# littlemesie/recommend-tf2.0

Measured on NVIDIA B200. Metric: DLRM train samples/sec, higher is better.
Workload: dtype f32

## Files before the change

recommend-tf2.0_b200/csrc/embed_bwd.cu:

```cuda
#include <cstdlib>

#include "rtf_common.cuh"

namespace rtf {

struct BwdParams {
  float* w[RTF_MAX_FIELDS];
  float* s1[RTF_MAX_FIELDS];
  float* s2[RTF_MAX_FIELDS];
  long long rows[RTF_MAX_FIELDS];
  int dim[RTF_MAX_FIELDS];
  int field_table[RTF_MAX_FIELDS];
  int field_off[RTF_MAX_FIELDS];
  int n_tables, n_fields, sumD, row_bits, L, pool;
  long long grad_sb;
  rtf_opt opt;
};

template <typename IdT>
__global__ void __launch_bounds__(256)
make_keys(const __grid_constant__ BwdParams P, const IdT* __restrict__ ids, long long n,
          long long sb, long long sf, long long sl, uint32_t* __restrict__ keys) {
  const long long p = (long long)blockIdx.x * blockDim.x + threadIdx.x;
  if (p >= n) return;
  const int F = P.n_fields;
  const long long LF = (long long)P.L * F;
  const long long b = p / LF;
  const int r = (int)(p - b * LF);
  const int l = r / F;
  const int f = r - l * F;
  const int t = P.field_table[f];
  const long long id = (long long)__ldg(ids + b * sb + (long long)f * sf + (long long)l * sl);
  uint32_t key;
  if (id < 0 || id >= P.rows[t])
    key = (uint32_t)P.n_tables << P.row_bits;
  else
    key = ((uint32_t)t << P.row_bits) | (uint32_t)id;
  keys[p] = key;
}

constexpr int SCAN_THREADS = 256;
constexpr int SCAN_ITEMS = 8;
constexpr int SCAN_TILE = SCAN_THREADS * SCAN_ITEMS;

template <typename T>
__device__ __forceinline__ T block_exclusive_scan(T v, T* total) {
  __shared__ T warp_tot[SCAN_THREADS / 32];
  const int lane = threadIdx.x & 31, wid = threadIdx.x >> 5;
  T inc = v;
#pragma unroll
  for (int o = 1; o < 32; o <<= 1) {
    T y = __shfl_up_sync(0xffffffffu, inc, o);
    if (lane >= o) inc += y;
  }
  if (lane == 31) warp_tot[wid] = inc;
  __syncthreads();
  T base = 0, tot = 0;
#pragma unroll
  for (int w = 0; w < SCAN_THREADS / 32; ++w) {
    const T t = warp_tot[w];
    if (w < wid) base += t;
    tot += t;
  }
  __syncthreads();
  *total = tot;
  return base + inc - v;
}

template <typename T, typename In>
__global__ void __launch_bounds__(SCAN_THREADS)
scan_tile_reduce(In in, long long n, T* __restrict__ tile_sums) {
  const long long base = (long long)blockIdx.x * SCAN_TILE + (long long)threadIdx.x * SCAN_ITEMS;
  T s = 0;
#pragma unroll
  for (int k = 0; k < SCAN_ITEMS; ++k)
    if (base + k < n) s += in(base + k);
  T tot;
  block_exclusive_scan<T>(s, &tot);
  if (threadIdx.x == 0) tile_sums[blockIdx.x] = tot;
}

template <typename T>
__global__ void __launch_bounds__(1024) scan_tile_sums(T* __restrict__ tile_sums, int nt) {
  __shared__ T wsum[32];
  __shared__ T carry_s;
  if (threadIdx.x == 0) carry_s = 0;
  __syncthreads();
  const int lane = threadIdx.x & 31, wid = threadIdx.x >> 5;
  for (int base = 0; base < nt; base += 1024) {
    const int i = base + threadIdx.x;
    const T v = i < nt ? tile_sums[i] : 0;
    T inc = v;
#pragma unroll
    for (int o = 1; o < 32; o <<= 1) {
      T y = __shfl_up_sync(0xffffffffu, inc, o);
      if (lane >= o) inc += y;
    }
    if (lane == 31) wsum[wid] = inc;
    __syncthreads();
    if (wid == 0) {
      T w = wsum[lane], winc = w;
#pragma unroll
      for (int o = 1; o < 32; o <<= 1) {
        T y = __shfl_up_sync(0xffffffffu, winc, o);
        if (lane >= o) winc += y;
      }
      wsum[lane] = winc - w;
    }
    __syncthreads();
    const T carry = carry_s;
    const T excl = carry + wsum[wid] + inc - v;
    if (i < nt) tile_sums[i] = excl;
    __syncthreads();
    if (threadIdx.x == 1023) carry_s = excl + v;
    __syncthreads();
  }
}

template <typename T, typename In, typename Out>
__global__ void __launch_bounds__(SCAN_THREADS)
scan_tile_apply(In in, Out out, long long n, const T* __restrict__ tile_sums) {
  const long long base = (long long)blockIdx.x * SCAN_TILE + (long long)threadIdx.x * SCAN_ITEMS;
  T v[SCAN_ITEMS];
  T s = 0;
#pragma unroll
  for (int k = 0; k < SCAN_ITEMS; ++k) {
    v[k] = base + k < n ? in(base + k) : 0;
    s += v[k];
  }
  T tot;
  T ex = block_exclusive_scan<T>(s, &tot) + tile_sums[blockIdx.x];
#pragma unroll
  for (int k = 0; k < SCAN_ITEMS; ++k) {
    if (base + k < n) out(base + k, ex, v[k]);
    ex += v[k];
  }
}

struct InArray {
  const uint32_t* a;
  __device__ uint32_t operator()(long long i) const { return a[i]; }
};
struct OutArray {
  uint32_t* a;
  __device__ void operator()(long long i, uint32_t ex, uint32_t) const { a[i] = ex; }
};
struct InHeadFlag {
  const uint32_t* keys;
  __device__ uint32_t operator()(long long i) const {
    return (i == 0 || keys[i] != keys[i - 1]) ? 1u : 0u;
  }
};
struct OutSegments {
  const uint32_t* keys;
  uint32_t* seg_start;
  int32_t* counters;
  int32_t* d_num_uniq;
  long long n;
  uint32_t sentinel_table;
  int row_bits;
  __device__ void operator()(long long i, uint32_t ex, uint32_t flag) const {
    if (flag) seg_start[ex] = (uint32_t)i;
    if (i == n - 1) {
      const uint32_t nseg = ex + flag;
      seg_start[nseg] = (uint32_t)n;
      const int valid = (int)nseg - ((keys[i] >> row_bits) == sentinel_table ? 1 : 0);
      counters[0] = (int)nseg;
      counters[1] = valid;
      if (d_num_uniq) *d_num_uniq = valid;
    }
  }
};

struct InSegKinds {
  const uint32_t* seg_start;
  const int32_t* counters;
  __device__ unsigned long long operator()(long long i) const {
    if (i >= counters[1]) return 0ull;
    const uint32_t len = seg_start[i + 1] - seg_start[i];
    if (len <= RTF_SEG_CHUNK) return 1ull;
    return (unsigned long long)((len + RTF_SEG_CHUNK - 1) / RTF_SEG_CHUNK) << 32;
  }
};
struct OutItems {
  const uint32_t* keys;
  const uint32_t* vals;
  const uint32_t* seg_start;
  int32_t* counters;
  uint4* items;
  uint32_t* short_seg;
  uint2* long_seg;
  uint32_t* arrive;
  uint32_t cap_chunk;
  __device__ void operator()(long long i, unsigned long long ex, unsigned long long v) const {
    const int n_valid = counters[1];
    if (i >= n_valid) return;
    const uint32_t start = seg_start[i], len = seg_start[i + 1] - start;
    const uint32_t key = keys[start];
    if (v & 0xffffffffull) {
      const uint32_t j = (uint32_t)ex;
      items[cap_chunk + j] = make_uint4(key, start, len, vals[start]);
      short_seg[j] = (uint32_t)i;
    } else {
      const uint32_t nch = (uint32_t)(v >> 32), slot0 = (uint32_t)(ex >> 32);
      long_seg[slot0] = make_uint2((uint32_t)i, nch);
      for (uint32_t c = 0; c < nch; ++c) {
        const uint32_t s = start + c * RTF_SEG_CHUNK;
        arrive[slot0 + c] = 0u;
        items[slot0 + c] = make_uint4(key, s, min((uint32_t)RTF_SEG_CHUNK, start + len - s), slot0);
      }
    }
    if (i == n_valid - 1) {
      const unsigned long long tot = ex + v;
      counters[2] = (int)(uint32_t)tot;
      counters[3] = (int)(uint32_t)(tot >> 32);
    }
  }
};

template <typename T, typename In, typename Out>
static int exclusive_scan(In in, Out out, long long n, T* tile_sums, cudaStream_t st) {
  const long long nt = (n + SCAN_TILE - 1) / SCAN_TILE;
  scan_tile_reduce<T, In><<<(unsigned)nt, SCAN_THREADS, 0, st>>>(in, n, tile_sums);
  scan_tile_sums<T><<<1, 1024, 0, st>>>(tile_sums, (int)nt);
  scan_tile_apply<T, In, Out><<<(unsigned)nt, SCAN_THREADS, 0, st>>>(in, out, n, tile_sums);
  RTF_CHECK_LAUNCH();
  return 0;
}

constexpr int SORT_THREADS = 256;
constexpr int SORT_WARPS = SORT_THREADS / 32;
constexpr int SORT_ITEMS = 16;
constexpr int SORT_TILE = SORT_THREADS * SORT_ITEMS;
constexpr int SORT_MAX_BITS = 10;
constexpr int SORT_MAX_BINS = 1 << SORT_MAX_BITS;

__global__ void __launch_bounds__(SORT_THREADS)
sort_hist(const uint32_t* __restrict__ keys, long long n, int shift, int bits,
          uint32_t* __restrict__ hist, int nblk) {
  __shared__ uint32_t sh[SORT_MAX_BINS];
  const int bins = 1 << bits;
  const uint32_t mask = (uint32_t)bins - 1u;
  for (int i = threadIdx.x; i < bins; i += SORT_THREADS) sh[i] = 0;
  __syncthreads();
  const long long base = (long long)blockIdx.x * SORT_TILE;
#pragma unroll
  for (int r = 0; r < SORT_ITEMS; ++r) {
    const long long i = base + r * SORT_THREADS + threadIdx.x;
    if (i < n) atomicAdd(&sh[(keys[i] >> shift) & mask], 1u);
  }
  __syncthreads();
  for (int d = threadIdx.x; d < bins; d += SORT_THREADS)
    hist[(long long)d * nblk + blockIdx.x] = sh[d];
}

__global__ void __launch_bounds__(SORT_THREADS)
sort_scatter(const uint32_t* __restrict__ keys_in, const uint32_t* __restrict__ vals_in,
             uint32_t* __restrict__ keys_out, uint32_t* __restrict__ vals_out, long long n,
             int shift, int bits, const uint32_t* __restrict__ hist_scanned, int nblk,
             int iota_vals) {
  __shared__ uint32_t whist[SORT_WARPS][SORT_MAX_BINS];
  const int bins = 1 << bits;
  const uint32_t mask = (uint32_t)bins - 1u;
  for (int i = threadIdx.x; i < SORT_WARPS * SORT_MAX_BINS; i += SORT_THREADS)
    (&whist[0][0])[i] = 0;
  __syncthreads();
  const int lane = threadIdx.x & 31, wid = threadIdx.x >> 5;
  const uint32_t lt_mask = (1u << lane) - 1u;
  const long long wbase = (long long)blockIdx.x * SORT_TILE + (long long)wid * (32 * SORT_ITEMS);
  uint32_t k[SORT_ITEMS], v[SORT_ITEMS], rank[SORT_ITEMS];
#pragma unroll
  for (int r = 0; r < SORT_ITEMS; ++r) {
    const long long i = wbase + r * 32 + lane;
    const bool valid = i < n;
    k[r] = valid ? keys_in[i] : 0xffffffffu;
    v[r] = valid ? (iota_vals ? (uint32_t)i : vals_in[i]) : 0u;
    const uint32_t vmask = __ballot_sync(0xffffffffu, valid);
    rank[r] = 0;
    if (valid) {
      const uint32_t d = (k[r] >> shift) & mask;
      const uint32_t m = __match_any_sync(vmask, d);
      const uint32_t prior = whist[wid][d];
      __syncwarp(vmask);
      if ((m & lt_mask) == 0) whist[wid][d] = prior + __popc(m);
      __syncwarp(vmask);
      rank[r] = prior + __popc(m & lt_mask);
    }
  }
  __syncthreads();
  for (int d = threadIdx.x; d < bins; d += SORT_THREADS) {
    uint32_t run = hist_scanned[(long long)d * nblk + blockIdx.x];
#pragma unroll
    for (int w = 0; w < SORT_WARPS; ++w) {
      const uint32_t c = whist[w][d];
      whist[w][d] = run;
      run += c;
    }
  }
  __syncthreads();
#pragma unroll
  for (int r = 0; r < SORT_ITEMS; ++r) {
    const long long i = wbase + r * 32 + lane;
    if (i < n) {
      const uint32_t d = (k[r] >> shift) & mask;
      const uint32_t pos = whist[wid][d] + rank[r];
      keys_out[pos] = k[r];
      vals_out[pos] = v[r];
    }
  }
}

template <int VEC>
struct Vec {
  float v[VEC];
};
template <int VEC>
__device__ __forceinline__ Vec<VEC> vload(const float* p) {
  Vec<VEC> r;
  if constexpr (VEC == 4) {
    const float4 t = *reinterpret_cast<const float4*>(p);
    r.v[0] = t.x; r.v[1] = t.y; r.v[2] = t.z; r.v[3] = t.w;
  } else {
    r.v[0] = *p;
  }
  return r;
}
template <int VEC>
__device__ __forceinline__ Vec<VEC> vload_stream(const float* p) {
  Vec<VEC> r;
  if constexpr (VEC == 4) {
    const float4 t = ldg_nc_f4(p);
    r.v[0] = t.x; r.v[1] = t.y; r.v[2] = t.z; r.v[3] = t.w;
  } else {
    r.v[0] = __ldg(p);
  }
  return r;
}
template <int VEC>
__device__ __forceinline__ void vstore(float* p, const Vec<VEC>& a) {
  if constexpr (VEC == 4)
    *reinterpret_cast<float4*>(p) = make_float4(a.v[0], a.v[1], a.v[2], a.v[3]);
  else
    *p = a.v[0];
}

__device__ __forceinline__ const float* grad_row(const BwdParams& P, const float* grad,
                                                 uint32_t p) {
  const int F = P.n_fields;
  const uint32_t LF = (uint32_t)P.L * (uint32_t)F;
  const uint32_t b = p / LF;
  const uint32_t r = p - b * LF;
  const uint32_t l = r / (uint32_t)F;
  const uint32_t f = r - l * (uint32_t)F;
  const long long lo = P.pool == RTF_POOL_NONE ? (long long)l * P.sumD : 0;
  return grad + (long long)b * P.grad_sb + lo + P.field_off[f];
}

template <int VEC, int G, int VPL>
__device__ __forceinline__ void sum_rows(const BwdParams& P, const float* __restrict__ grad,
                                         const uint32_t* __restrict__ vals, uint32_t start,
                                         uint32_t end, bool have_first, uint32_t first_pos, int nv,
                                         int lg, float scale, Vec<VEC> (&acc)[VPL]) {
  constexpr int U = 4;
#pragma unroll 1
  for (uint32_t j0 = start; j0 < end; j0 += U) {
    const float* src[U];
#pragma unroll
    for (int u = 0; u < U; ++u) {
      src[u] = nullptr;
      if (j0 + u < end) {
        const uint32_t p = (have_first && j0 + u == start) ? first_pos : __ldg(vals + j0 + u);
        src[u] = grad_row(P, grad, p);
      }
    }
    Vec<VEC> x[U][VPL];
#pragma unroll
    for (int u = 0; u < U; ++u)
#pragma unroll
      for (int k = 0; k < VPL; ++k) {
        const int vi = lg + k * G;
        if (src[u] && vi < nv) x[u][k] = vload_stream<VEC>(src[u] + VEC * vi);
      }
#pragma unroll
    for (int u = 0; u < U; ++u)
      if (src[u]) {
#pragma unroll
        for (int k = 0; k < VPL; ++k) {
          const int vi = lg + k * G;
          if (vi < nv) {
#pragma unroll
// ... 197 lines not shown
  for (int k = 0; k < VPL; ++k)
#pragma unroll
    for (int e = 0; e < VEC; ++e) acc[k].v[e] = 0.f;
  if (i >= n_chunk) {
    RowState<VEC, VPL> st;
    if (len <= 2) {
      load_row_state<VEC, G, VPL>(P, key, nv, lg, st);
      const float* r0 = grad_row(P, grad, rec.w);
      const float* r1 = len == 2 ? grad_row(P, grad, __ldg(S.vals + start + 1)) : nullptr;
      Vec<VEC> x0[VPL], x1[VPL];
#pragma unroll
      for (int k = 0; k < VPL; ++k) {
        const int vi = lg + k * G;
        if (vi < nv) {
          x0[k] = vload_stream<VEC>(r0 + VEC * vi);
          if (r1) x1[k] = vload_stream<VEC>(r1 + VEC * vi);
        }
      }
#pragma unroll
      for (int k = 0; k < VPL; ++k) {
        const int vi = lg + k * G;
        if (vi < nv) {
#pragma unroll
          for (int e = 0; e < VEC; ++e) {
            float g = x0[k].v[e];
            if (P.pool == RTF_POOL_MEAN) g = __fmul_rn(g, scale);
            acc[k].v[e] = __fadd_rn(acc[k].v[e], g);
            if (r1) {
              float h = x1[k].v[e];
              if (P.pool == RTF_POOL_MEAN) h = __fmul_rn(h, scale);
              acc[k].v[e] = __fadd_rn(acc[k].v[e], h);
            }
          }
        }
      }
    } else {
      sum_rows<VEC, G, VPL>(P, grad, S.vals, start, start + len, true, rec.w, nv, lg, scale, acc);
      load_row_state<VEC, G, VPL>(P, key, nv, lg, st);
    }
    uint32_t seg = 0;
    if (S.uniq_key || S.uniq_grad) seg = __ldg(S.short_seg + (i - n_chunk));
    finish_row<VEC, G, VPL>(P, key, seg, nv, lg, acc, st, S.uniq_key, S.uniq_grad, S.dim_max);
    return;
  }
  const int g0 = (int)(threadIdx.x & 31) / G * G;
  const uint32_t gmask = G == 32 ? 0xffffffffu : (((1u << (G & 31)) - 1u) << g0);
  const uint32_t slot0 = rec.w;
  sum_rows<VEC, G, VPL>(P, grad, S.vals, start, start + len, false, 0u, nv, lg, scale, acc);
#pragma unroll
  for (int k = 0; k < VPL; ++k) {
    const int vi = lg + k * G;
    if (vi < nv) vstore<VEC>(S.partials + (long long)i * S.dim_max + VEC * vi, acc[k]);
  }
  __threadfence();
  __syncwarp(gmask);
  const uint2 ls = __ldg(S.long_seg + slot0);
  if (ls.y <= RTF_SEG_GROUP) {
    uint32_t ticket = 0;
    if (lg == 0) ticket = atomicAdd(S.arrive + slot0, 1u);
    ticket = __shfl_sync(gmask, ticket, g0);
    if (ticket != ls.y - 1) return;
  }
  combine_long<VEC, G, VPL>(P, S, key, slot0, i - slot0, ls, nv, lg, gmask, g0);
}

template <int VEC, int G, int VPL, int MINB>
static int launch_apply(const BwdParams& P, const SegWork& S, const float* grad,
                        long long max_items, cudaStream_t st) {
  const long long blocks = (max_items * G + 255) / 256;
  seg_apply<VEC, G, VPL, MINB><<<(unsigned)blocks, 256, 0, st>>>(P, S, grad);
  RTF_CHECK_LAUNCH();
  return 0;
}

template <int VEC, int G, int VPL>
static int launch_segments(const BwdParams& P, const SegWork& S, const float* grad,
                           long long max_items, cudaStream_t st) {
  return launch_apply<VEC, G, VPL, (VPL == 1 ? 8 : 4)>(P, S, grad, max_items, st);
}

static inline size_t align_up(size_t x, size_t a) { return (x + a - 1) / a * a; }

struct WsLayout {
  size_t keys0, keys1, vals0, vals1, hist, tile_sums, seg_start, counters, items, short_seg,
      long_seg, arrive, partials, total;
  size_t cap_chunk;
};
static WsLayout ws_layout(long long n, int dim_max) {
  WsLayout w;
  const size_t nn = (size_t)(n > 0 ? n : 1);
  const size_t nblk = (nn + SORT_TILE - 1) / SORT_TILE;
  size_t o = 0;
  auto take = [&](size_t bytes) { size_t r = o; o = align_up(o + bytes, 256); return r; };
  w.keys0 = take(nn * 4);
  w.keys1 = take(nn * 4);
  w.vals0 = take(nn * 4);
  w.vals1 = take(nn * 4);
  w.hist = take((size_t)SORT_MAX_BINS * nblk * 4);
  const size_t scan_n = nn > (size_t)SORT_MAX_BINS * nblk ? nn : (size_t)SORT_MAX_BINS * nblk;
  w.tile_sums = take(((scan_n + SCAN_TILE - 1) / SCAN_TILE + 1) * 8);
  w.seg_start = take((nn + 1) * 4);
  w.counters = take(16);
  w.cap_chunk = 2 * nn / RTF_SEG_CHUNK + 4;
  w.items = take((w.cap_chunk + nn) * 16);
  w.short_seg = take(nn * 4);
  w.long_seg = take(w.cap_chunk * 8);
  w.arrive = take(w.cap_chunk * 4);
  w.partials = take(w.cap_chunk * (size_t)dim_max * 4);
  w.total = o;
  return w;
}

}

extern "C" int rtf_embed_bwd_workspace(int64_t n_lookups, int dim_max, size_t* bytes) {
  if (!bytes || n_lookups < 0 || dim_max <= 0) return RTF_E_ARG;
  *bytes = rtf::ws_layout(n_lookups, dim_max).total;
  return 0;
}

static int embed_bwd_impl(int phase, float* const* weights, float* const* state1,
                          float* const* state2, const int64_t* rows, const int32_t* dims,
                          int n_tables, const int32_t* field_table, int n_fields,
                          const void* d_ids, int ids_i64, int64_t B, int L, int64_t ids_sb,
                          int64_t ids_sf, int64_t ids_sl, int pool, const float* d_grad,
                          int64_t grad_sb, const rtf_opt* opt, uint32_t* d_uniq_key,
                          float* d_uniq_grad, int32_t* d_num_uniq, int* row_bits_out,
                          void* d_workspace, size_t workspace_bytes, void* stream) {
  using namespace rtf;
  static const rtf_opt kNoOpt = {RTF_OPT_NONE, 0.f, 0.f, 0.f, 0.f, 0.f, nullptr};
  static float* const kNoPtrs[RTF_MAX_FIELDS] = {};
  if (!(phase & 2)) {
    opt = &kNoOpt;
    weights = kNoPtrs;
    state1 = state2 = nullptr;
  }
  if (!weights || !rows || !dims || !field_table || !opt) return RTF_E_ARG;
  if (n_tables <= 0 || n_fields <= 0 || B < 0 || L <= 0) return RTF_E_ARG;
  if (B > 0 && !d_workspace) return RTF_E_ARG;
  if (B > 0 && (phase & 1) && !d_ids) return RTF_E_ARG;
  if (B > 0 && (phase & 2) && !d_grad) return RTF_E_ARG;
  if (n_tables > RTF_MAX_FIELDS || n_fields > RTF_MAX_FIELDS) return RTF_E_RANGE;
  if (pool < RTF_POOL_NONE || pool > RTF_POOL_MEAN) return RTF_E_ARG;
  if (opt->kind < RTF_OPT_NONE || opt->kind > RTF_OPT_ADAM) return RTF_E_ARG;
  cudaStream_t st = (cudaStream_t)stream;

  BwdParams P;
  long long rows_max = 1;
  int dim_max = 0;
  bool vec_ok = ((uintptr_t)d_grad % 16 == 0) && (grad_sb % 4 == 0) &&
                (!d_uniq_grad || (uintptr_t)d_uniq_grad % 16 == 0);
  for (int t = 0; t < n_tables; ++t) {
    if (rows[t] <= 0 || dims[t] <= 0) return RTF_E_ARG;
    P.w[t] = weights[t];
    P.s1[t] = state1 ? state1[t] : nullptr;
    P.s2[t] = state2 ? state2[t] : nullptr;
    P.rows[t] = rows[t];
    P.dim[t] = dims[t];
    if (opt->kind != RTF_OPT_NONE && !P.w[t]) return RTF_E_ARG;
    if (opt->kind >= RTF_OPT_ADAGRAD && !P.s1[t]) return RTF_E_ARG;
    if (opt->kind == RTF_OPT_ADAM && !P.s2[t]) return RTF_E_ARG;
    if (dims[t] % 4 || (uintptr_t)P.w[t] % 16 || (uintptr_t)P.s1[t] % 16 ||
        (uintptr_t)P.s2[t] % 16)
      vec_ok = false;
    if (rows[t] > rows_max) rows_max = rows[t];
    if (dims[t] > dim_max) dim_max = dims[t];
  }
  int off = 0;
  for (int f = 0; f < n_fields; ++f) {
    const int t = field_table[f];
    if (t < 0 || t >= n_tables) return RTF_E_ARG;
    P.field_table[f] = t;
    P.field_off[f] = off;
    if (off % 4) vec_ok = false;
    off += dims[t];
  }
  P.sumD = off;
  if (off % 4) vec_ok = false;
  int row_bits = 1;
  while (((long long)1 << row_bits) < rows_max) ++row_bits;
  int table_bits = 1;
  while ((1 << table_bits) < n_tables + 1) ++table_bits;
  if (row_bits + table_bits > 32) return RTF_E_RANGE;
  if (row_bits_out) *row_bits_out = row_bits;
  P.n_tables = n_tables;
  P.n_fields = n_fields;
  P.row_bits = row_bits;
  P.L = L;
  P.pool = pool;
  P.grad_sb = grad_sb;
  P.opt = *opt;

  const long long n = B * (long long)L * n_fields;
  if (n >= 0x7fffffffLL) return RTF_E_RANGE;
  if (n == 0) {
    if (d_num_uniq) cudaMemsetAsync(d_num_uniq, 0, 4, st);
    return 0;
  }
  if (dim_max > (vec_ok ? 512 : 128)) return RTF_E_RANGE;
  const WsLayout W = ws_layout(n, dim_max);
  if (workspace_bytes < W.total) return RTF_E_WORKSPACE;
  if ((uintptr_t)d_workspace % 256) return RTF_E_ALIGN;
  char* ws = (char*)d_workspace;
  uint32_t* keys[2] = {(uint32_t*)(ws + W.keys0), (uint32_t*)(ws + W.keys1)};
  uint32_t* vals[2] = {(uint32_t*)(ws + W.vals0), (uint32_t*)(ws + W.vals1)};
  uint32_t* hist = (uint32_t*)(ws + W.hist);
  uint32_t* tile_sums = (uint32_t*)(ws + W.tile_sums);
  uint32_t* seg_start = (uint32_t*)(ws + W.seg_start);
  int32_t* counters = (int32_t*)(ws + W.counters);

  const int nblk = (int)((n + SORT_TILE - 1) / SORT_TILE);
  const int total_bits = row_bits + table_bits;
  const int npass = (total_bits + SORT_MAX_BITS - 1) / SORT_MAX_BITS;
  const int bits = (total_bits + npass - 1) / npass;
  int cur = npass & 1;
  if (phase & 1) {
  cur = 0;
  const unsigned kb = (unsigned)((n + 255) / 256);
  if (ids_i64)
    make_keys<int64_t><<<kb, 256, 0, st>>>(P, (const int64_t*)d_ids, n, ids_sb, ids_sf, ids_sl,
                                           keys[0]);
  else
    make_keys<int32_t><<<kb, 256, 0, st>>>(P, (const int32_t*)d_ids, n, ids_sb, ids_sf, ids_sl,
                                           keys[0]);
  RTF_CHECK_LAUNCH();

  for (int shift = 0, pass = 0; pass < npass; shift += bits, ++pass) {
    sort_hist<<<nblk, SORT_THREADS, 0, st>>>(keys[cur], n, shift, bits, hist, nblk);
    int rc = exclusive_scan<uint32_t>(InArray{hist}, OutArray{hist}, (long long)(1 << bits) * nblk,
                                      tile_sums, st);
    if (rc) return rc;
    sort_scatter<<<nblk, SORT_THREADS, 0, st>>>(keys[cur], vals[cur], keys[cur ^ 1],
                                                vals[cur ^ 1], n, shift, bits, hist, nblk,
                                                pass == 0);
    RTF_CHECK_LAUNCH();
    cur ^= 1;
  }

  cudaError_t ce = cudaMemsetAsync(counters, 0, 16, st);
  if (ce != cudaSuccess) return (int)ce;
  {
    OutSegments outseg{keys[cur], seg_start, counters, d_num_uniq, n, (uint32_t)n_tables,
                       row_bits};
    int rc = exclusive_scan<uint32_t>(InHeadFlag{keys[cur]}, outseg, n, tile_sums, st);
    if (rc) return rc;
  }
  {
    OutItems outit{keys[cur], vals[cur], seg_start, counters, (uint4*)(ws + W.items),
                   (uint32_t*)(ws + W.short_seg), (uint2*)(ws + W.long_seg),
                   (uint32_t*)(ws + W.arrive), (uint32_t)W.cap_chunk};
    int rc = exclusive_scan<unsigned long long>(InSegKinds{seg_start, counters}, outit, n,
                                                (unsigned long long*)tile_sums, st);
    if (rc) return rc;
  }
  }
  if (!(phase & 2)) return 0;

  SegWork S;
  S.vals = vals[cur];
  S.counters = counters;
  S.items = (const uint4*)(ws + W.items);
  S.short_seg = (const uint32_t*)(ws + W.short_seg);
  S.long_seg = (const uint2*)(ws + W.long_seg);
  S.arrive = (uint32_t*)(ws + W.arrive);
  S.partials = (float*)(ws + W.partials);
  S.uniq_key = d_uniq_key;
  S.uniq_grad = d_uniq_grad;
  S.cap_chunk = (uint32_t)W.cap_chunk;
  S.dim_max = dim_max;

  long long max_items = 0;
  {
    long long per_table[RTF_MAX_FIELDS] = {};
    for (int f = 0; f < n_fields; ++f) per_table[field_table[f]] += B * (long long)L;
    for (int t = 0; t < n_tables; ++t) {
      const long long nt = per_table[t];
      const long long b = rows[t] + 2 * (nt / RTF_SEG_CHUNK) + 2;
      max_items += nt < b ? nt : b;
    }
    if (max_items > n) max_items = n;
    if (max_items < 1) max_items = 1;
  }
  if (vec_ok) {
    const int nv = dim_max / 4;
    int G = 1;
    while (G < nv && G < 32) G <<= 1;
    const int vpl = (nv + G - 1) / G;
    if (vpl == 1) {
      switch (G) {
        case 1: return launch_segments<4, 1, 1>(P, S, d_grad, max_items, st);
        case 2: return launch_segments<4, 2, 1>(P, S, d_grad, max_items, st);
        case 4: return launch_segments<4, 4, 1>(P, S, d_grad, max_items, st);
        case 8: return launch_segments<4, 8, 1>(P, S, d_grad, max_items, st);
        case 16: return launch_segments<4, 16, 1>(P, S, d_grad, max_items, st);
        default: return launch_segments<4, 32, 1>(P, S, d_grad, max_items, st);
      }
    }
    if (vpl == 2) return launch_segments<4, 32, 2>(P, S, d_grad, max_items, st);
    return launch_segments<4, 32, 4>(P, S, d_grad, max_items, st);
  }
  {
    int G = 1;
    while (G < dim_max && G < 32) G <<= 1;
    const int vpl = (dim_max + G - 1) / G;
    if (vpl == 1) {
      switch (G) {
        case 1: return launch_segments<1, 1, 1>(P, S, d_grad, max_items, st);
        case 2: return launch_segments<1, 2, 1>(P, S, d_grad, max_items, st);
        case 4: return launch_segments<1, 4, 1>(P, S, d_grad, max_items, st);
        case 8: return launch_segments<1, 8, 1>(P, S, d_grad, max_items, st);
        case 16: return launch_segments<1, 16, 1>(P, S, d_grad, max_items, st);
        default: return launch_segments<1, 32, 1>(P, S, d_grad, max_items, st);
      }
    }
    if (vpl == 2) return launch_segments<1, 32, 2>(P, S, d_grad, max_items, st);
    return launch_segments<1, 32, 4>(P, S, d_grad, max_items, st);
  }
}

extern "C" int rtf_embed_bwd(float* const* weights, float* const* state1, float* const* state2,
                             const int64_t* rows, const int32_t* dims, int n_tables,
                             const int32_t* field_table, int n_fields, const void* d_ids,
                             int ids_i64, int64_t B, int L, int64_t ids_sb, int64_t ids_sf,
                             int64_t ids_sl, int pool, const float* d_grad, int64_t grad_sb,
                             const rtf_opt* opt, uint32_t* d_uniq_key, float* d_uniq_grad,
                             int32_t* d_num_uniq, int* row_bits_out, void* d_workspace,
                             size_t workspace_bytes, void* stream) {
  return embed_bwd_impl(3, weights, state1, state2, rows, dims, n_tables, field_table, n_fields,
                        d_ids, ids_i64, B, L, ids_sb, ids_sf, ids_sl, pool, d_grad, grad_sb, opt,
                        d_uniq_key, d_uniq_grad, d_num_uniq, row_bits_out, d_workspace,
                        workspace_bytes, stream);
}

extern "C" int rtf_embed_bwd_prepare(const int64_t* rows, const int32_t* dims, int n_tables,
                                     const int32_t* field_table, int n_fields, const void* d_ids,
                                     int ids_i64, int64_t B, int L, int64_t ids_sb, int64_t ids_sf,
                                     int64_t ids_sl, int32_t* d_num_uniq, int* row_bits_out,
// ... 19 lines not shown
```

Before: 8.909 million.

## Replace multi-kernel radix sort and scans with onesweep decoupled-lookback sort

Replaces the per-pass histogram, three-kernel scan and scatter radix sort with a single upfront key-build-plus-all-pass histogram kernel, followed by one onesweep kernel per pass that uses decoupled lookback with tile tickets. The two segment-building scans are fused into one seg_items kernel that does head/tail detection and item emission with chained tile prefixes. Digit width drops from 10 to 8 bits. The aim is to cut kernel launches and global passes over keys in the embedding-backward sort. The cost is spin-waiting lookback, more passes from the narrower digits, and correctness that depends on forward-progress ordering.

```diff
diff --git a/recommend-tf2.0_b200/csrc/embed_bwd.cu b/recommend-tf2.0_b200/csrc/embed_bwd.cu
--- a/recommend-tf2.0_b200/csrc/embed_bwd.cu
+++ b/recommend-tf2.0_b200/csrc/embed_bwd.cu
@@ -17,257 +17,185 @@
   rtf_opt opt;
 };
 
-template <typename IdT>
-__global__ void __launch_bounds__(256)
-make_keys(const __grid_constant__ BwdParams P, const IdT* __restrict__ ids, long long n,
-          long long sb, long long sf, long long sl, uint32_t* __restrict__ keys) {
-  const long long p = (long long)blockIdx.x * blockDim.x + threadIdx.x;
-  if (p >= n) return;
-  const int F = P.n_fields;
-  const long long LF = (long long)P.L * F;
-  const long long b = p / LF;
-  const int r = (int)(p - b * LF);
-  const int l = r / F;
-  const int f = r - l * F;
-  const int t = P.field_table[f];
-  const long long id = (long long)__ldg(ids + b * sb + (long long)f * sf + (long long)l * sl);
-  uint32_t key;
-  if (id < 0 || id >= P.rows[t])
-    key = (uint32_t)P.n_tables << P.row_bits;
-  else
-    key = ((uint32_t)t << P.row_bits) | (uint32_t)id;
-  keys[p] = key;
-}
-
-constexpr int SCAN_THREADS = 256;
-constexpr int SCAN_ITEMS = 8;
-constexpr int SCAN_TILE = SCAN_THREADS * SCAN_ITEMS;
-
-template <typename T>
-__device__ __forceinline__ T block_exclusive_scan(T v, T* total) {
-  __shared__ T warp_tot[SCAN_THREADS / 32];
-  const int lane = threadIdx.x & 31, wid = threadIdx.x >> 5;
-  T inc = v;
-#pragma unroll
-  for (int o = 1; o < 32; o <<= 1) {
-    T y = __shfl_up_sync(0xffffffffu, inc, o);
-    if (lane >= o) inc += y;
-  }
-  if (lane == 31) warp_tot[wid] = inc;
-  __syncthreads();
-  T base = 0, tot = 0;
-#pragma unroll
-  for (int w = 0; w < SCAN_THREADS / 32; ++w) {
-    const T t = warp_tot[w];
-    if (w < wid) base += t;
-    tot += t;
-  }
-  __syncthreads();
-  *total = tot;
-  return base + inc - v;
-}
-
-template <typename T, typename In>
-__global__ void __launch_bounds__(SCAN_THREADS)
-scan_tile_reduce(In in, long long n, T* __restrict__ tile_sums) {
-  const long long base = (long long)blockIdx.x * SCAN_TILE + (long long)threadIdx.x * SCAN_ITEMS;
-  T s = 0;
-#pragma unroll
-  for (int k = 0; k < SCAN_ITEMS; ++k)
-    if (base + k < n) s += in(base + k);
-  T tot;
-  block_exclusive_scan<T>(s, &tot);
-  if (threadIdx.x == 0) tile_sums[blockIdx.x] = tot;
-}
-
-template <typename T>
-__global__ void __launch_bounds__(1024) scan_tile_sums(T* __restrict__ tile_sums, int nt) {
-  __shared__ T wsum[32];
-  __shared__ T carry_s;
-  if (threadIdx.x == 0) carry_s = 0;
-  __syncthreads();
-  const int lane = threadIdx.x & 31, wid = threadIdx.x >> 5;
-  for (int base = 0; base < nt; base += 1024) {
-    const int i = base + threadIdx.x;
-    const T v = i < nt ? tile_sums[i] : 0;
-    T inc = v;
-#pragma unroll
-    for (int o = 1; o < 32; o <<= 1) {
-      T y = __shfl_up_sync(0xffffffffu, inc, o);
-      if (lane >= o) inc += y;
-    }
-    if (lane == 31) wsum[wid] = inc;
-    __syncthreads();
-    if (wid == 0) {
-      T w = wsum[lane], winc = w;
-#pragma unroll
-      for (int o = 1; o < 32; o <<= 1) {
-        T y = __shfl_up_sync(0xffffffffu, winc, o);
-        if (lane >= o) winc += y;
-      }
-      wsum[lane] = winc - w;
-    }
-    __syncthreads();
-    const T carry = carry_s;
-    const T excl = carry + wsum[wid] + inc - v;
-    if (i < nt) tile_sums[i] = excl;
-    __syncthreads();
-    if (threadIdx.x == 1023) carry_s = excl + v;
-    __syncthreads();
-  }
-}
-
-template <typename T, typename In, typename Out>
-__global__ void __launch_bounds__(SCAN_THREADS)
-scan_tile_apply(In in, Out out, long long n, const T* __restrict__ tile_sums) {
-  const long long base = (long long)blockIdx.x * SCAN_TILE + (long long)threadIdx.x * SCAN_ITEMS;
-  T v[SCAN_ITEMS];
-  T s = 0;
-#pragma unroll
-  for (int k = 0; k < SCAN_ITEMS; ++k) {
-    v[k] = base + k < n ? in(base + k) : 0;
-    s += v[k];
-  }
-  T tot;
-  T ex = block_exclusive_scan<T>(s, &tot) + tile_sums[blockIdx.x];
-#pragma unroll
-  for (int k = 0; k < SCAN_ITEMS; ++k) {
-    if (base + k < n) out(base + k, ex, v[k]);
-    ex += v[k];
-  }
-}
-
-struct InArray {
-  const uint32_t* a;
-  __device__ uint32_t operator()(long long i) const { return a[i]; }
-};
-struct OutArray {
-  uint32_t* a;
-  __device__ void operator()(long long i, uint32_t ex, uint32_t) const { a[i] = ex; }
-};
-struct InHeadFlag {
-  const uint32_t* keys;
-  __device__ uint32_t operator()(long long i) const {
-    return (i == 0 || keys[i] != keys[i - 1]) ? 1u : 0u;
-  }
-};
-struct OutSegments {
-  const uint32_t* keys;
-  uint32_t* seg_start;
-  int32_t* counters;
-  int32_t* d_num_uniq;
-  long long n;
-  uint32_t sentinel_table;
-  int row_bits;
-  __device__ void operator()(long long i, uint32_t ex, uint32_t flag) const {
-    if (flag) seg_start[ex] = (uint32_t)i;
-    if (i == n - 1) {
-      const uint32_t nseg = ex + flag;
-      seg_start[nseg] = (uint32_t)n;
-      const int valid = (int)nseg - ((keys[i] >> row_bits) == sentinel_table ? 1 : 0);
-      counters[0] = (int)nseg;
-      counters[1] = valid;
-      if (d_num_uniq) *d_num_uniq = valid;
-    }
-  }
-};
-
-struct InSegKinds {
-  const uint32_t* seg_start;
-  const int32_t* counters;
-  __device__ unsigned long long operator()(long long i) const {
-    if (i >= counters[1]) return 0ull;
-    const uint32_t len = seg_start[i + 1] - seg_start[i];
-    if (len <= RTF_SEG_CHUNK) return 1ull;
-    return (unsigned long long)((len + RTF_SEG_CHUNK - 1) / RTF_SEG_CHUNK) << 32;
-  }
-};
-struct OutItems {
-  const uint32_t* keys;
-  const uint32_t* vals;
-  const uint32_t* seg_start;
-  int32_t* counters;
-  uint4* items;
-  uint32_t* short_seg;
-  uint2* long_seg;
-  uint32_t* arrive;
-  uint32_t cap_chunk;
-  __device__ void operator()(long long i, unsigned long long ex, unsigned long long v) const {
-    const int n_valid = counters[1];
-    if (i >= n_valid) return;
-    const uint32_t start = seg_start[i], len = seg_start[i + 1] - start;
-    const uint32_t key = keys[start];
-    if (v & 0xffffffffull) {
-      const uint32_t j = (uint32_t)ex;
-      items[cap_chunk + j] = make_uint4(key, start, len, vals[start]);
-      short_seg[j] = (uint32_t)i;
-    } else {
-      const uint32_t nch = (uint32_t)(v >> 32), slot0 = (uint32_t)(ex >> 32);
-      long_seg[slot0] = make_uint2((uint32_t)i, nch);
-      for (uint32_t c = 0; c < nch; ++c) {
-        const uint32_t s = start + c * RTF_SEG_CHUNK;
-        arrive[slot0 + c] = 0u;
-        items[slot0 + c] = make_uint4(key, s, min((uint32_t)RTF_SEG_CHUNK, start + len - s), slot0);
-      }
-    }
-    if (i == n_valid - 1) {
-      const unsigned long long tot = ex + v;
-      counters[2] = (int)(uint32_t)tot;
-      counters[3] = (int)(uint32_t)(tot >> 32);
-    }
-  }
-};
-
-template <typename T, typename In, typename Out>
-static int exclusive_scan(In in, Out out, long long n, T* tile_sums, cudaStream_t st) {
-  const long long nt = (n + SCAN_TILE - 1) / SCAN_TILE;
-  scan_tile_reduce<T, In><<<(unsigned)nt, SCAN_THREADS, 0, st>>>(in, n, tile_sums);
-  scan_tile_sums<T><<<1, 1024, 0, st>>>(tile_sums, (int)nt);
-  scan_tile_apply<T, In, Out><<<(unsigned)nt, SCAN_THREADS, 0, st>>>(in, out, n, tile_sums);
-  RTF_CHECK_LAUNCH();
-  return 0;
-}
-
 constexpr int SORT_THREADS = 256;
 constexpr int SORT_WARPS = SORT_THREADS / 32;
 constexpr int SORT_ITEMS = 16;
 constexpr int SORT_TILE = SORT_THREADS * SORT_ITEMS;
-constexpr int SORT_MAX_BITS = 10;
+constexpr int SORT_MAX_BITS = 8;
+constexpr int LOOKBACK = 12;
 constexpr int SORT_MAX_BINS = 1 << SORT_MAX_BITS;
-
-__global__ void __launch_bounds__(SORT_THREADS)
-sort_hist(const uint32_t* __restrict__ keys, long long n, int shift, int bits,
-          uint32_t* __restrict__ hist, int nblk) {
-  __shared__ uint32_t sh[SORT_MAX_BINS];
+constexpr int SORT_MAX_PASSES = (32 + SORT_MAX_BITS - 1) / SORT_MAX_BITS;
+constexpr int KEYS_THREADS = 256;
+constexpr int KEYS_ITEMS = 8;
+
+static inline void sort_plan(int total_bits, int* npass, int* bits) {
+  *npass = (total_bits + SORT_MAX_BITS - 1) / SORT_MAX_BITS;
+  *bits = (total_bits + *npass - 1) / *npass;
+}
+
+__device__ __forceinline__ uint32_t ld_relaxed(const uint32_t* p) {
+  uint32_t v;
+  asm volatile("ld.relaxed.gpu.global.u32 %0, [%1];" : "=r"(v) : "l"(p) : "memory");
+  return v;
+}
+__device__ __forceinline__ void st_relaxed(uint32_t* p, uint32_t v) {
+  asm volatile("st.relaxed.gpu.global.u32 [%0], %1;" ::"l"(p), "r"(v) : "memory");
+}
+__device__ __forceinline__ unsigned long long ld_relaxed(const unsigned long long* p) {
+  unsigned long long v;
+  asm volatile("ld.relaxed.gpu.global.u64 %0, [%1];" : "=l"(v) : "l"(p) : "memory");
+  return v;
+}
+__device__ __forceinline__ void st_relaxed(unsigned long long* p, unsigned long long v) {
+  asm volatile("st.relaxed.gpu.global.u64 [%0], %1;" ::"l"(p), "l"(v) : "memory");
+}
+
+template <typename Op>
+__device__ __forceinline__ uint2 block_exclusive_scan(uint2 v, uint2* total, Op op) {
+  __shared__ uint2 warp_tot[SORT_WARPS];
+  const int lane = threadIdx.x & 31, wid = threadIdx.x >> 5;
+  uint2 inc = v;
+#pragma unroll
+  for (int o = 1; o < 32; o <<= 1) {
+    const uint2 y = make_uint2(__shfl_up_sync(0xffffffffu, inc.x, o),
+                               __shfl_up_sync(0xffffffffu, inc.y, o));
+    if (lane >= o) inc = op(y, inc);
+  }
+  uint2 ex = make_uint2(__shfl_up_sync(0xffffffffu, inc.x, 1), __shfl_up_sync(0xffffffffu, inc.y, 1));
+  if (lane == 0) ex = make_uint2(0u, 0u);
+  if (lane == 31) warp_tot[wid] = inc;
+  __syncthreads();
+  uint2 base = make_uint2(0u, 0u), tot = make_uint2(0u, 0u);
+#pragma unroll
+  for (int w = 0; w < SORT_WARPS; ++w) {
+    const uint2 t = warp_tot[w];
+    if (w < wid) base = op(base, t);
+    tot = op(tot, t);
+  }
+  __syncthreads();
+  *total = tot;
+  return op(base, ex);
+}
+struct SumOp {
+  __device__ uint2 operator()(uint2 a, uint2 b) const { return make_uint2(a.x + b.x, a.y + b.y); }
+};
+struct SumMaxOp {
+  __device__ uint2 operator()(uint2 a, uint2 b) const { return make_uint2(a.x + b.x, max(a.y, b.y)); }
+};
+
+constexpr unsigned long long ST_AGG = 1ull << 62, ST_INC = 2ull << 62;
+__device__ __forceinline__ unsigned long long st_pack(uint2 v) {
+  return ((unsigned long long)v.x << 31) | v.y;
+}
+__device__ __forceinline__ uint2 st_unpack(unsigned long long s) {
+  return make_uint2((uint32_t)(s >> 31) & 0x7fffffffu, (uint32_t)s & 0x7fffffffu);
+}
+
+template <typename Op>
+__device__ __forceinline__ uint2 tile_prefix(unsigned long long* status, uint32_t tile, uint2 agg,
+                                             Op op) {
+  __shared__ uint2 pre_s;
+  if (tile == 0) {
+    if (threadIdx.x == 0) st_relaxed(status, ST_INC | st_pack(agg));
+    return make_uint2(0u, 0u);
+  }
+  if (threadIdx.x < 32) {
+    const int lane = threadIdx.x;
+    if (lane == 0) st_relaxed(status + tile, ST_AGG | st_pack(agg));
+    uint2 pre = make_uint2(0u, 0u);
+    for (long long t = (long long)tile - 1;; t -= 32) {
+      unsigned long long s = ST_INC;
+      if (t - lane >= 0) {
+        do s = ld_relaxed(status + (t - lane)); while ((s >> 62) == 0);
+      }
+      const uint32_t inc = __ballot_sync(0xffffffffu, (s >> 62) == 2);
+      const int stop = inc ? __ffs(inc) - 1 : 31;
+      uint2 v = lane <= stop ? st_unpack(s) : make_uint2(0u, 0u);
+#pragma unroll
+      for (int o = 16; o > 0; o >>= 1)
+        v = op(v, make_uint2(__shfl_xor_sync(0xffffffffu, v.x, o),
+                             __shfl_xor_sync(0xffffffffu, v.y, o)));
+      pre = op(pre, v);
+      if (inc) break;
+    }
+    if (lane == 0) {
+      st_relaxed(status + tile, ST_INC | st_pack(op(pre, agg)));
+      pre_s = pre;
+    }
+  }
+  __syncthreads();
+  return pre_s;
+}
+
+template <typename IdT>
+__global__ void __launch_bounds__(KEYS_THREADS)
+sort_keys_hist(const __grid_constant__ BwdParams P, const IdT* __restrict__ ids, long long n,
+               long long sb, long long sf, long long sl, int npass, int bits,
+               uint32_t* __restrict__ keys, uint32_t* __restrict__ ghist) {
+  __shared__ uint32_t sh[SORT_MAX_PASSES * SORT_MAX_BINS];
   const int bins = 1 << bits;
   const uint32_t mask = (uint32_t)bins - 1u;
-  for (int i = threadIdx.x; i < bins; i += SORT_THREADS) sh[i] = 0;
+  for (int i = threadIdx.x; i < npass * bins; i += KEYS_THREADS) sh[i] = 0;
   __syncthreads();
-  const long long base = (long long)blockIdx.x * SORT_TILE;
-#pragma unroll
-  for (int r = 0; r < SORT_ITEMS; ++r) {
-    const long long i = base + r * SORT_THREADS + threadIdx.x;
-    if (i < n) atomicAdd(&sh[(keys[i] >> shift) & mask], 1u);
+  const uint32_t F = (uint32_t)P.n_fields;
+  const uint32_t LF = (uint32_t)P.L * F;
+  for (long long p0 = (long long)blockIdx.x * (KEYS_THREADS * KEYS_ITEMS); p0 < n;
+       p0 += (long long)gridDim.x * (KEYS_THREADS * KEYS_ITEMS)) {
+    long long id[KEYS_ITEMS];
+    int tb[KEYS_ITEMS];
+#pragma unroll
+    for (int j = 0; j < KEYS_ITEMS; ++j) {
+      const uint32_t p = (uint32_t)(p0 + j * KEYS_THREADS + threadIdx.x);
+      tb[j] = -1;
+      if (p < n) {
+        const uint32_t b = p / LF, r = p - b * LF;
+        const uint32_t l = r / F, f = r - l * F;
+        tb[j] = P.field_table[f];
+        id[j] = (long long)__ldg(ids + (long long)b * sb + (long long)f * sf + (long long)l * sl);
+      }
+    }
+#pragma unroll
+    for (int j = 0; j < KEYS_ITEMS; ++j) {
+      if (tb[j] < 0) continue;
+      const int t = tb[j];
+      uint32_t key;
+      if (id[j] < 0 || id[j] >= P.rows[t])
+        key = (uint32_t)P.n_tables << P.row_bits;
+      else
+        key = ((uint32_t)t << P.row_bits) | (uint32_t)id[j];
+      keys[p0 + j * KEYS_THREADS + threadIdx.x] = key;
+      for (int s = 0; s < npass; ++s) atomicAdd(&sh[s * bins + ((key >> (s * bits)) & mask)], 1u);
+    }
   }
   __syncthreads();
-  for (int d = threadIdx.x; d < bins; d += SORT_THREADS)
-    hist[(long long)d * nblk + blockIdx.x] = sh[d];
+  for (int i = threadIdx.x; i < npass * bins; i += KEYS_THREADS)
+    if (sh[i]) atomicAdd(ghist + i, sh[i]);
 }
 
 __global__ void __launch_bounds__(SORT_THREADS)
-sort_scatter(const uint32_t* __restrict__ keys_in, const uint32_t* __restrict__ vals_in,
-             uint32_t* __restrict__ keys_out, uint32_t* __restrict__ vals_out, long long n,
-             int shift, int bits, const uint32_t* __restrict__ hist_scanned, int nblk,
-             int iota_vals) {
+sort_onesweep(const uint32_t* __restrict__ keys_in, const uint32_t* __restrict__ vals_in,
+              uint32_t* __restrict__ keys_out, uint32_t* __restrict__ vals_out, long long n,
+              int shift, int bits, const uint32_t* __restrict__ ghist, uint32_t* status,
+              uint32_t* ticket, int iota_vals) {
+  static_assert(SORT_MAX_BINS == SORT_THREADS, "one digit per thread");
   __shared__ uint32_t whist[SORT_WARPS][SORT_MAX_BINS];
+  __shared__ uint32_t s_key[SORT_TILE], s_val[SORT_TILE];
+  __shared__ uint32_t s_goff[SORT_MAX_BINS];
+  __shared__ uint32_t tile_s;
   const int bins = 1 << bits;
   const uint32_t mask = (uint32_t)bins - 1u;
+  const int d = threadIdx.x;
+  if (threadIdx.x == 0) tile_s = atomicAdd(ticket, 1u);
   for (int i = threadIdx.x; i < SORT_WARPS * SORT_MAX_BINS; i += SORT_THREADS)
     (&whist[0][0])[i] = 0;
-  __syncthreads();
+  uint2 tot;
+  const uint32_t gex =
+      block_exclusive_scan(make_uint2(d < bins ? __ldg(ghist + d) : 0u, 0u), &tot, SumOp()).x;
+  const uint32_t tile = tile_s;
+
   const int lane = threadIdx.x & 31, wid = threadIdx.x >> 5;
   const uint32_t lt_mask = (1u << lane) - 1u;
-  const long long wbase = (long long)blockIdx.x * SORT_TILE + (long long)wid * (32 * SORT_ITEMS);
+  const long long wbase = (long long)tile * SORT_TILE + (long long)wid * (32 * SORT_ITEMS);
   uint32_t k[SORT_ITEMS], v[SORT_ITEMS], rank[SORT_ITEMS];
 #pragma unroll
   for (int r = 0; r < SORT_ITEMS; ++r) {
@@ -278,34 +206,178 @@
     const uint32_t vmask = __ballot_sync(0xffffffffu, valid);
     rank[r] = 0;
     if (valid) {
-      const uint32_t d = (k[r] >> shift) & mask;
-      const uint32_t m = __match_any_sync(vmask, d);
-      const uint32_t prior = whist[wid][d];
+      const uint32_t dr = (k[r] >> shift) & mask;
+      const uint32_t m = __match_any_sync(vmask, dr);
+      const uint32_t prior = whist[wid][dr];
       __syncwarp(vmask);
-      if ((m & lt_mask) == 0) whist[wid][d] = prior + __popc(m);
+      if ((m & lt_mask) == 0) whist[wid][dr] = prior + __popc(m);
       __syncwarp(vmask);
       rank[r] = prior + __popc(m & lt_mask);
     }
   }
   __syncthreads();
-  for (int d = threadIdx.x; d < bins; d += SORT_THREADS) {
-    uint32_t run = hist_scanned[(long long)d * nblk + blockIdx.x];
+  uint32_t cnt = 0;
+  uint32_t* my = status + (size_t)tile * bins;
+  if (d < bins) {
 #pragma unroll
     for (int w = 0; w < SORT_WARPS; ++w) {
       const uint32_t c = whist[w][d];
-      whist[w][d] = run;
-      run += c;
-    }
+      whist[w][d] = cnt;
+      cnt += c;
+    }
+    st_relaxed(my + d, (tile == 0 ? 0x80000000u : 0u) | (cnt + 1u));
+  }
+  const uint32_t tile_off = block_exclusive_scan(make_uint2(cnt, 0u), &tot, SumOp()).x;
+  uint32_t excl = 0;
+  if (tile > 0 && d < bins) {
+    int t = (int)tile - 1;
+    bool done = false;
+    while (!done) {
+      uint32_t s[LOOKBACK];
+#pragma unroll
+      for (int w = 0; w < LOOKBACK; ++w)
+        s[w] = t - w < 0 ? 0x80000001u : ld_relaxed(status + (size_t)(t - w) * bins + d);
+      bool stop = false;
+#pragma unroll
+      for (int w = 0; w < LOOKBACK; ++w) {
+        const uint32_t x = s[w];
+        if (stop) continue;
+        if (x == 0) {
+          stop = true;
+        } else {
+          excl += (x & 0x7fffffffu) - 1u;
+          if (x >> 31) done = stop = true;
+          else --t;
+        }
+      }
+    }
+    st_relaxed(my + d, 0x80000000u | (excl + cnt + 1u));
+  }
+  if (d < bins) {
+    s_goff[d] = gex + excl - tile_off;
+#pragma unroll
+    for (int w = 0; w < SORT_WARPS; ++w) whist[w][d] += tile_off;
   }
   __syncthreads();
 #pragma unroll
   for (int r = 0; r < SORT_ITEMS; ++r) {
-    const long long i = wbase + r * 32 + lane;
-    if (i < n) {
-      const uint32_t d = (k[r] >> shift) & mask;
-      const uint32_t pos = whist[wid][d] + rank[r];
-      keys_out[pos] = k[r];
-      vals_out[pos] = v[r];
+    if (wbase + r * 32 + lane < n) {
+      const uint32_t pos = whist[wid][(k[r] >> shift) & mask] + rank[r];
+      s_key[pos] = k[r];
+      s_val[pos] = v[r];
+    }
+  }
+  __syncthreads();
+  const long long left = n - (long long)tile * SORT_TILE;
+  const int tile_n = left < SORT_TILE ? (int)left : SORT_TILE;
+  for (int i = threadIdx.x; i < tile_n; i += SORT_THREADS) {
+    const uint32_t key = s_key[i];
+    const uint32_t pos = (uint32_t)i + s_goff[(key >> shift) & mask];
+    keys_out[pos] = key;
+    vals_out[pos] = s_val[i];
+  }
+}
+
+__global__ void __launch_bounds__(SORT_THREADS)
+seg_items(const uint32_t* __restrict__ keys, const uint32_t* __restrict__ vals, long long n_ll,
+          uint32_t sentinel_table, int row_bits, uint32_t cap_chunk, int ntiles,
+          unsigned long long* status, uint32_t* ticket, uint32_t* __restrict__ seg_start,
+          int32_t* __restrict__ counters, int32_t* __restrict__ d_num_uniq,
+          uint4* __restrict__ items, uint32_t* __restrict__ short_seg,
+          uint2* __restrict__ long_seg, uint32_t* __restrict__ arrive) {
+  constexpr uint32_t CH = RTF_SEG_CHUNK;
+  __shared__ uint32_t tile_s;
+  if (threadIdx.x == 0) tile_s = atomicAdd(ticket, 1u);
+  __syncthreads();
+  const uint32_t tile = tile_s;
+  const uint32_t n = (uint32_t)n_ll;
+  const uint32_t q0 = tile * SORT_TILE + threadIdx.x * SORT_ITEMS;
+  uint32_t k[SORT_ITEMS];
+  if (q0 + SORT_ITEMS <= n) {
+#pragma unroll
+    for (int j = 0; j < SORT_ITEMS; j += 4) {
+      const uint4 t = __ldg(reinterpret_cast<const uint4*>(keys + q0 + j));
+      k[j] = t.x; k[j + 1] = t.y; k[j + 2] = t.z; k[j + 3] = t.w;
+    }
+  } else {
+#pragma unroll
+    for (int j = 0; j < SORT_ITEMS; ++j) k[j] = q0 + j < n ? __ldg(keys + q0 + j) : 0xffffffffu;
+  }
+  const uint32_t prev = q0 > 0 && q0 < n ? __ldg(keys + q0 - 1) : ~k[0];
+  const uint32_t next = q0 + SORT_ITEMS < n ? __ldg(keys + q0 + SORT_ITEMS) : ~k[SORT_ITEMS - 1];
+  uint32_t headm = 0, tailm = 0;
+#pragma unroll
+  for (int j = 0; j < SORT_ITEMS; ++j) {
+    const uint32_t q = q0 + j;
+    if (q < n) {
+      if (k[j] != (j > 0 ? k[j - 1] : prev)) headm |= 1u << j;
+      if (q + 1 == n || k[j] != (j + 1 < SORT_ITEMS ? k[j + 1] : next)) tailm |= 1u << j;
+    }
+  }
+  const uint2 aggA = make_uint2(__popc(headm), headm ? q0 + 31 - __clz(headm) : 0u);
+  uint2 totA;
+  const uint2 exA = block_exclusive_scan(aggA, &totA, SumMaxOp());
+  const uint2 runA0 = SumMaxOp()(tile_prefix(status, tile, totA, SumMaxOp()), exA);
+  uint2 aggB = make_uint2(0u, 0u);
+  {
+    uint32_t start = runA0.y;
+#pragma unroll
+    for (int j = 0; j < SORT_ITEMS; ++j) {
+      if (headm >> j & 1u) start = q0 + j;
+      if ((tailm >> j & 1u) && (k[j] >> row_bits) != sentinel_table) {
+        const uint32_t len = q0 + j - start + 1;
+        if (len <= CH) aggB.x += 1;
+        else aggB.y += (len + CH - 1) / CH;
+      }
+    }
+  }
+  uint2 totB;
+  const uint2 exB = block_exclusive_scan(aggB, &totB, SumOp());
+  uint2 runB = SumOp()(tile_prefix(status + ntiles, tile, totB, SumOp()), exB);
+
+  uint2 runA = runA0;
+  const int last_tail = tailm ? 31 - __clz(tailm) : -1;
+#pragma unroll
+  for (int j = 0; j < SORT_ITEMS; ++j) {
+    const uint32_t q = q0 + j;
+    if (q >= n) break;
+    const uint32_t key = k[j];
+    if (headm >> j & 1u) {
+      seg_start[runA.x] = q;
+      runA = make_uint2(runA.x + 1, q);
+    }
+    const uint32_t start = runA.y;
+    const bool valid = (key >> row_bits) != sentinel_table;
+    if (valid) {
+      if ((q - start) % CH == 0 && j > last_tail && q + CH < n && __ldg(keys + q + CH) == key) {
+        const uint32_t slot0 = runB.y, c = (q - start) / CH;
+        items[slot0 + c] = make_uint4(key, q, CH, slot0);
+        arrive[slot0 + c] = 0u;
+      }
+      if (tailm >> j & 1u) {
+        const uint32_t len = q - start + 1, seg = runA.x - 1;
+        if (len <= CH) {
+          items[cap_chunk + runB.x] = make_uint4(key, start, len, __ldg(vals + start));
+          short_seg[runB.x] = seg;
+          runB.x += 1;
+        } else {
+          const uint32_t nch = (len + CH - 1) / CH, slot0 = runB.y, c = nch - 1;
+          items[slot0 + c] = make_uint4(key, start + c * CH, len - c * CH, slot0);
+          arrive[slot0 + c] = 0u;
+          long_seg[slot0] = make_uint2(seg, nch);
+          runB.y += nch;
+        }
+      }
+    }
+    if (q == n - 1) {
+      const uint32_t nseg = runA.x;
+      seg_start[nseg] = n;
+      const int n_valid = (int)nseg - (valid ? 0 : 1);
+      counters[0] = (int)nseg;
+      counters[1] = n_valid;
+      counters[2] = (int)runB.x;
+      counters[3] = (int)runB.y;
+      if (d_num_uniq) *d_num_uniq = n_valid;
     }
   }
 }
@@ -669,23 +741,24 @@
 static inline size_t align_up(size_t x, size_t a) { return (x + a - 1) / a * a; }
 
 struct WsLayout {
-  size_t keys0, keys1, vals0, vals1, hist, tile_sums, seg_start, counters, items, short_seg,
-      long_seg, arrive, partials, total;
+  size_t keys0, keys1, vals0, vals1, ghist, tickets, seg_status, sort_status, seg_start, counters,
+      items, short_seg, long_seg, arrive, partials, total;
   size_t cap_chunk;
 };
 static WsLayout ws_layout(long long n, int dim_max) {
   WsLayout w;
   const size_t nn = (size_t)(n > 0 ? n : 1);
-  const size_t nblk = (nn + SORT_TILE - 1) / SORT_TILE;
+  const size_t ntiles = (nn + SORT_TILE - 1) / SORT_TILE;
   size_t o = 0;
   auto take = [&](size_t bytes) { size_t r = o; o = align_up(o + bytes, 256); return r; };
   w.keys0 = take(nn * 4);
   w.keys1 = take(nn * 4);
   w.vals0 = take(nn * 4);
   w.vals1 = take(nn * 4);
-  w.hist = take((size_t)SORT_MAX_BINS * nblk * 4);
-  const size_t scan_n = nn > (size_t)SORT_MAX_BINS * nblk ? nn : (size_t)SORT_MAX_BINS * nblk;
-  w.tile_sums = take(((scan_n + SCAN_TILE - 1) / SCAN_TILE + 1) * 8);
+  w.ghist = take((size_t)SORT_MAX_PASSES * SORT_MAX_BINS * 4);
+  w.tickets = take((SORT_MAX_PASSES + 1) * 4);
+  w.seg_status = take(2 * ntiles * 8);
+  w.sort_status = take((size_t)SORT_MAX_PASSES * ntiles * SORT_MAX_BINS * 4);
   w.seg_start = take((nn + 1) * 4);
   w.counters = take(16);
   w.cap_chunk = 2 * nn / RTF_SEG_CHUNK + 4;
@@ -791,55 +864,47 @@
   char* ws = (char*)d_workspace;
   uint32_t* keys[2] = {(uint32_t*)(ws + W.keys0), (uint32_t*)(ws + W.keys1)};
   uint32_t* vals[2] = {(uint32_t*)(ws + W.vals0), (uint32_t*)(ws + W.vals1)};
-  uint32_t* hist = (uint32_t*)(ws + W.hist);
-  uint32_t* tile_sums = (uint32_t*)(ws + W.tile_sums);
   uint32_t* seg_start = (uint32_t*)(ws + W.seg_start);
   int32_t* counters = (int32_t*)(ws + W.counters);
 
-  const int nblk = (int)((n + SORT_TILE - 1) / SORT_TILE);
-  const int total_bits = row_bits + table_bits;
-  const int npass = (total_bits + SORT_MAX_BITS - 1) / SORT_MAX_BITS;
-  const int bits = (total_bits + npass - 1) / npass;
+  const int ntiles = (int)((n + SORT_TILE - 1) / SORT_TILE);
+  int npass, bits;
+  sort_plan(row_bits + table_bits, &npass, &bits);
   int cur = npass & 1;
   if (phase & 1) {
-  cur = 0;
-  const unsigned kb = (unsigned)((n + 255) / 256);
-  if (ids_i64)
-    make_keys<int64_t><<<kb, 256, 0, st>>>(P, (const int64_t*)d_ids, n, ids_sb, ids_sf, ids_sl,
-                                           keys[0]);
-  else
-    make_keys<int32_t><<<kb, 256, 0, st>>>(P, (const int32_t*)d_ids, n, ids_sb, ids_sf, ids_sl,
-                                           keys[0]);
-  RTF_CHECK_LAUNCH();
-
-  for (int shift = 0, pass = 0; pass < npass; shift += bits, ++pass) {
-    sort_hist<<<nblk, SORT_THREADS, 0, st>>>(keys[cur], n, shift, bits, hist, nblk);
-    int rc = exclusive_scan<uint32_t>(InArray{hist}, OutArray{hist}, (long long)(1 << bits) * nblk,
-                                      tile_sums, st);
-    if (rc) return rc;
-    sort_scatter<<<nblk, SORT_THREADS, 0, st>>>(keys[cur], vals[cur], keys[cur ^ 1],
-                                                vals[cur ^ 1], n, shift, bits, hist, nblk,
-                                                pass == 0);
+    const int bins = 1 << bits;
+    uint32_t* ghist = (uint32_t*)(ws + W.ghist);
+    uint32_t* tickets = (uint32_t*)(ws + W.tickets);
+    uint32_t* sort_status = (uint32_t*)(ws + W.sort_status);
+    cudaError_t ce = cudaMemsetAsync(ws + W.ghist, 0,
+                                     W.sort_status - W.ghist + (size_t)npass * ntiles * bins * 4, st);
+    if (ce != cudaSuccess) return (int)ce;
+    const long long kt = (n + KEYS_THREADS * KEYS_ITEMS - 1) / (KEYS_THREADS * KEYS_ITEMS);
+    const unsigned kb = (unsigned)(kt < 2 * kNumSMs ? kt : 2 * kNumSMs);
+    if (ids_i64)
+      sort_keys_hist<int64_t><<<kb, KEYS_THREADS, 0, st>>>(P, (const int64_t*)d_ids, n, ids_sb,
+                                                           ids_sf, ids_sl, npass, bits, keys[0],
+                                                           ghist);
+    else
+      sort_keys_hist<int32_t><<<kb, KEYS_THREADS, 0, st>>>(P, (const int32_t*)d_ids, n, ids_sb,
+                                                           ids_sf, ids_sl, npass, bits, keys[0],
+                                                           ghist);
     RTF_CHECK_LAUNCH();
-    cur ^= 1;
-  }
-
-  cudaError_t ce = cudaMemsetAsync(counters, 0, 16, st);
-  if (ce != cudaSuccess) return (int)ce;
-  {
-    OutSegments outseg{keys[cur], seg_start, counters, d_num_uniq, n, (uint32_t)n_tables,
-                       row_bits};
-    int rc = exclusive_scan<uint32_t>(InHeadFlag{keys[cur]}, outseg, n, tile_sums, st);
-    if (rc) return rc;
-  }
-  {
-    OutItems outit{keys[cur], vals[cur], seg_start, counters, (uint4*)(ws + W.items),
-                   (uint32_t*)(ws + W.short_seg), (uint2*)(ws + W.long_seg),
-                   (uint32_t*)(ws + W.arrive), (uint32_t)W.cap_chunk};
-    int rc = exclusive_scan<unsigned long long>(InSegKinds{seg_start, counters}, outit, n,
-                                                (unsigned long long*)tile_sums, st);
-    if (rc) return rc;
-  }
+    cur = 0;
+    for (int pass = 0; pass < npass; ++pass) {
+      sort_onesweep<<<ntiles, SORT_THREADS, 0, st>>>(
+          keys[cur], vals[cur], keys[cur ^ 1], vals[cur ^ 1], n, pass * bits, bits,
+          ghist + pass * bins, sort_status + (size_t)pass * ntiles * bins, tickets + pass,
+          pass == 0);
+      RTF_CHECK_LAUNCH();
+      cur ^= 1;
+    }
+    seg_items<<<ntiles, SORT_THREADS, 0, st>>>(
+        keys[cur], vals[cur], n, (uint32_t)n_tables, row_bits, (uint32_t)W.cap_chunk, ntiles,
+        (unsigned long long*)(ws + W.seg_status), tickets + SORT_MAX_PASSES, seg_start, counters,
+        d_num_uniq, (uint4*)(ws + W.items), (uint32_t*)(ws + W.short_seg),
+        (uint2*)(ws + W.long_seg), (uint32_t*)(ws + W.arrive));
+    RTF_CHECK_LAUNCH();
   }
   if (!(phase & 2)) return 0;
 
```

Result: no change. 8.843 million (median of 6 runs) (-0.7%).
